# lucidrains/magvit2-pytorch

Hardware: NVIDIA H100
Metric: video-frames/sec tokenize+decode, 17x128x128 bf16 (higher is better)
Workload: dtype bf16

## Files before the change

### magvit2_pytorch_b200/csrc/tc_slab.cu

```cuda
#include "common.cuh"
#include "tc_common.cuh"
#include <cuda.h>
#include <algorithm>
#include <type_traits>
#include <mutex>
#include <map>
#include <vector>
#include <string.h>

namespace mv2 {

struct alignas(64) SlabParams {
  CUtensorMap amap;
  CUtensorMap hmap;
  CUtensorMap wmap;
  CUtensorMap wmap2;
  int kt, kh, kw, pt, ph, pw;
  int st;
  int hist_T;
  int Ci, kchunks, row_bytes;
  int B, T, H, W, Co;
  int mw, pitch, slab_h, slab_bytes, slab_stride;
  int bn, n_tiles_n, tiles_w, tiles_h, total_tiles;
  int slab_stages, w_stages;
  int tpw;
  TcEpi epi;
  CUtensorMap w1map;
  const float* bias1;
  const float* se_wk;
  float se_bk;
  float* se_ws;
  CUtensorMap amap_odd;
  int dn_e_off;
  int dn_aoff[6];
  int dn_lower;
  int h_stride;
  CUtensorMap ymap;
  CUtensorMap rmap;
};

__host__ __device__ constexpr bool slab_tma_epi(int mode) {
  return mode == EPI_PLAIN || mode == EPI_PLAIN_RES || mode == EPI_GEGLU || mode == EPI_DOWN_SPACE;
}
__host__ __device__ constexpr int slab_out_box_ch(int mode, int bn) {
  return (mode == EPI_GEGLU ? bn / 2 : bn) < 64 ? (mode == EPI_GEGLU ? bn / 2 : bn) : 64;
}

__host__ __device__ __forceinline__ void slab_frame_of(const SlabParams& p, int slot, int& b, int& t) {
  const int ptc = p.pt > 0 ? (p.pt + p.st - 1) / p.st : 0;
  const int n_cheap = ptc < p.T ? ptc : p.T, n_full = p.T - n_cheap;
  const int full_slots = p.B * n_full;
  if (slot < full_slots) { b = slot / n_full; t = n_cheap + slot - b * n_full; }
  else { const int r = slot - full_slots; const int level = r / p.B; b = r - level * p.B; t = n_cheap - 1 - level; }
}
__host__ __device__ __forceinline__ int slab_tile_of_cta(const SlabParams& p, int k, int cta, int grid) {
  const int tile = k * grid + ((k & 1) ? grid - 1 - cta : cta);
  return tile < p.total_tiles ? tile : -1;
}
__device__ __forceinline__ int slab_tile_of(const SlabParams& p, int k) { return slab_tile_of_cta(p, k, blockIdx.x, gridDim.x); }

struct TileCoord { int b, t, h0, w0, n0; };
__host__ __device__ __forceinline__ TileCoord decode_tile(const SlabParams& p, int tile) {
  TileCoord c;
  const int nt = tile % p.n_tiles_n; tile /= p.n_tiles_n;
  const int tw = tile % p.tiles_w; tile /= p.tiles_w;
  const int th = tile % p.tiles_h; tile /= p.tiles_h;
  slab_frame_of(p, tile, c.b, c.t);
  c.h0 = th * 16;
  c.w0 = tw * 8 * p.mw;
  c.n0 = nt * p.bn;
  return c;
}

struct SlabSmem { uint32_t sbias, stage0, lpart, accstg, hbuf, end, rbar, otile, rtile; };
__host__ __device__ __forceinline__ SlabSmem slab_smem_layout(const SlabParams& p, uint32_t bar0, bool fused) {
  SlabSmem m;
  m.sbias = (bar0 + 8 * (2 * p.slab_stages + 2 * p.w_stages) + 15) & ~15u;
  m.stage0 = m.sbias + (uint32_t)(p.n_tiles_n * p.bn) * 4 * (fused ? 3 : 1);
  m.lpart = m.stage0 + (fused ? 0 : 8 * 2048);
  m.accstg = m.lpart + (fused ? 2048 : 0);
  m.hbuf = m.accstg + 2u * p.mw * 64 * (p.bn + 4) * 4;
  if (fused) m.hbuf = (m.hbuf + 1023u) & ~1023u;
  m.end = m.hbuf + (fused ? (uint32_t)p.h_stride : 0);
  m.rbar = m.stage0;
  m.otile = (m.rbar + 32 + 1023u) & ~1023u;
  m.rtile = m.otile + 2u * p.mw * 64 * p.bn * 2;
  return m;
}

template <int MODE, int BN, int ACT, int MWMAX>
__device__ __forceinline__ void slab_epi_fragment(const SlabParams& p, const float (&acc)[MWMAX][BN / 2], const TileCoord& c,
                                                  const float* sbias, uint32_t ot, uint32_t rt, int wq, int lane, bool relu) {
  constexpr int OC = MODE == EPI_GEGLU ? BN / 2 : BN, CB = slab_out_box_ch(MODE, BN), NB = OC / CB;
  constexpr uint32_t RB = CB * 2, BOX = 64 * RB, SWZ = (RB / 16 - 1) << 4;
  const uint32_t m0 = 16 * wq + (lane >> 2), q4 = (lane & 3) * 4;
  auto at = [&](int j, int col, uint32_t m) {
    const uint32_t off = m * RB + (uint32_t)(col % CB) * 2 + q4;
    return (uint32_t)(j * NB + col / CB) * BOX + (off ^ ((off >> 3) & SWZ));
  };
  auto st32 = [](uint32_t a, uint32_t v) { asm volatile("st.shared.b32 [%0], %1;" ::"r"(a), "r"(v) : "memory"); };
  const float* os = (MODE == EPI_PLAIN || MODE == EPI_PLAIN_RES) && p.epi.oscale ? p.epi.oscale + (int64_t)c.b * p.Co : nullptr;
  const float rs = MODE == EPI_PLAIN_RES && p.epi.mode == 2 ? 0.70710678118654752440f : 1.f;
#pragma unroll
  for (int j = 0; j < MWMAX; ++j) {
    if (j >= p.mw) break;
    if (MODE == EPI_GEGLU) {
#pragma unroll
      for (int g = 0; g < BN / 16; ++g) {
        const int n = c.n0 + 16 * g + 2 * (lane & 3);
        const float2 bx = *reinterpret_cast<const float2*>(sbias + n), bg = *reinterpret_cast<const float2*>(sbias + n + 8);
#pragma unroll
        for (int hr = 0; hr < 2; ++hr) {
          const float* xv = &acc[j][8 * g + 2 * hr];
          const float* gv = &acc[j][8 * g + 4 + 2 * hr];
          const float v0 = gelu_fast(gv[0] + bg.x) * (xv[0] + bx.x);
          const float v1 = gelu_fast(gv[1] + bg.y) * (xv[1] + bx.y);
          st32(ot + at(j, 8 * g, m0 + 8 * hr), pack_bf16x2(v0, v1));
        }
      }
    } else {
#pragma unroll
      for (int g = 0; g < BN / 8; ++g) {
        const int col = 8 * g, n = c.n0 + col + 2 * (lane & 3);
        const float2 b = *reinterpret_cast<const float2*>(sbias + n);
        float o0 = 1.f, o1 = 1.f;
        if (os) { o0 = n < p.Co ? os[n] : 0.f; o1 = n + 1 < p.Co ? os[n + 1] : 0.f; }
#pragma unroll
        for (int hr = 0; hr < 2; ++hr) {
          float v0 = acc[j][4 * g + 2 * hr], v1 = acc[j][4 * g + 2 * hr + 1];
          if (os) { v0 *= o0; v1 *= o1; }
          v0 = act_ct<ACT>(v0 + b.x, relu);
          v1 = act_ct<ACT>(v1 + b.y, relu);
          const uint32_t a = at(j, col, m0 + 8 * hr);
          if (MODE == EPI_PLAIN_RES) {
            uint32_t r;
            asm volatile("ld.shared.b32 %0, [%1];" : "=r"(r) : "r"(rt + a) : "memory");
            v0 = (v0 + __uint_as_float(r << 16)) * rs;
            v1 = (v1 + __uint_as_float(r & 0xffff0000u)) * rs;
          }
          st32(ot + a, pack_bf16x2(v0, v1));
        }
      }
    }
  }
}

constexpr int SLAB_PRODUCER_REGS = 40, SLAB_CONSUMER_REGS = 232;
template <int MODE, int BN>
__global__ void __launch_bounds__(384, 1) tc_slab_kernel(const __grid_constant__ SlabParams p) {
  constexpr int MWMAX = BN >= 32 ? 128 / BN : 4;
  constexpr int KC1 = BN >= 64 ? BN / 64 : 1;
  extern __shared__ uint8_t smem_raw[];
  const uint32_t smem_base = (smem_u32(smem_raw) + 1023u) & ~1023u;
  const int warp = threadIdx.x >> 5, lane = threadIdx.x & 31;
  const uint32_t row_bytes = p.row_bytes;
  const uint32_t bk = row_bytes >> 1;
  const uint32_t w_tile = p.bn * row_bytes;
  const uint32_t w_bytes = w_tile * p.tpw;
  const uint32_t slab0 = smem_base;
  const uint32_t wst0 = smem_base + p.slab_stages * p.slab_stride;
  const uint32_t bar0 = wst0 + p.w_stages * w_bytes;
  const uint32_t slab_full = bar0, slab_empty = slab_full + 8 * p.slab_stages;
  const uint32_t w_full = slab_empty + 8 * p.slab_stages, w_empty = w_full + 8 * p.w_stages;
  const SlabSmem L = slab_smem_layout(p, bar0, MODE == EPI_FUSED_RU);
  auto gen = [&](uint32_t u) { return smem_raw + (u - smem_u32(smem_raw)); };
  float* sbias = reinterpret_cast<float*>(gen(L.sbias));
  const uint32_t nbias = (uint32_t)(p.n_tiles_n * p.bn);
  const uint32_t stage0 = L.stage0;

  if (threadIdx.x == 0) {
    for (int s = 0; s < p.slab_stages; ++s) { mbar_init(slab_full + 8 * s, 1); mbar_init(slab_empty + 8 * s, 8); }
    for (int s = 0; s < p.w_stages; ++s) { mbar_init(w_full + 8 * s, 1); mbar_init(w_empty + 8 * s, 8); }
    if (MODE == EPI_PLAIN_RES)
      for (int g = 0; g < 2; ++g) { mbar_init(L.rbar + 8 * g, 1); mbar_init(L.rbar + 16 + 8 * g, 4); }
    fence_barrier_init();
  }
  if (warp == 0 && lane == 0) {
    tma_prefetch_desc(&p.amap);
    if (MODE == EPI_DOWN_SPACE) tma_prefetch_desc(&p.amap_odd);
    else if (p.hist_T > 0) tma_prefetch_desc(&p.hmap);
  }
  if (warp == 2 && lane == 0) {
    tma_prefetch_desc(&p.wmap); tma_prefetch_desc(&p.wmap2);
    if (MODE == EPI_FUSED_RU) tma_prefetch_desc(&p.w1map);
  }
  if (slab_tma_epi(MODE) && warp == 1 && lane == 0) {
    tma_prefetch_desc(&p.ymap);
    if (MODE == EPI_PLAIN_RES) tma_prefetch_desc(&p.rmap);
  }
  if (warp >= 4) {
    const int nb = p.n_tiles_n * p.bn;
    for (int i = threadIdx.x - 128; i < nb; i += 256) sbias[i] = (p.epi.bias && i < p.Co) ? p.epi.bias[i] : 0.f;
    if (MODE == EPI_FUSED_RU)
      for (int i = threadIdx.x - 128; i < nb; i += 256) {
        sbias[nb + i] = (p.bias1 && i < p.Co) ? p.bias1[i] : 0.f;
        sbias[2 * nb + i] = i < p.Co ? p.se_wk[i] : 0.f;
      }
  }
  __syncthreads();
  pdl_wait();
  pdl_launch_dependents();

  const int taps2d = p.kh * p.kw;

  if (warp < 4) {
    setmaxnreg_dec<SLAB_PRODUCER_REGS>();
    if (warp == 0) {
      if (MODE == EPI_DOWN_SPACE) {
        if (lane == 0) {
          uint32_t s = 0, ph = 0;
          for (int tk = 0, tile; (tile = slab_tile_of(p, tk)) >= 0; ++tk) {
            const TileCoord c = decode_tile(p, tile);
            for (int kc = 0; kc < p.kchunks; ++kc) {
              mbar_wait(slab_empty + 8 * s, ph ^ 1);
              mbar_expect_tx(slab_full + 8 * s, p.slab_bytes);
              tma_load_5d(slab0 + s * p.slab_stride, &p.amap_odd, slab_full + 8 * s, kc * bk, c.w0 - 1, c.h0 - 1, c.t, c.b);
              tma_load_5d(slab0 + s * p.slab_stride + p.dn_e_off, &p.amap, slab_full + 8 * s, kc * bk, c.w0 - 1, c.h0, c.t, c.b);
              if (++s == (uint32_t)p.slab_stages) { s = 0; ph ^= 1; }
            }
          }
        }
      } else
      if (lane == 0) {
        uint32_t s = 0, ph = 0;
        for (int tk = 0, tile; (tile = slab_tile_of(p, tk)) >= 0; ++tk) {
          const TileCoord c = decode_tile(p, tile);
          const int dt0 = max(0, p.pt - c.t * p.st - p.hist_T);
          for (int dt = dt0; dt < p.kt; ++dt)
            for (int kc = 0; kc < p.kchunks; ++kc) {
              mbar_wait(slab_empty + 8 * s, ph ^ 1);
              mbar_expect_tx(slab_full + 8 * s, p.slab_bytes);
              const int ti = c.t * p.st + dt - p.pt;
              tma_load_5d(slab0 + s * p.slab_stride, ti >= 0 ? &p.amap : &p.hmap, slab_full + 8 * s, kc * bk, c.w0 - p.pw,
                          c.h0 - p.ph, ti >= 0 ? ti : ti + p.hist_T, c.b);
              if (++s == (uint32_t)p.slab_stages) { s = 0; ph ^= 1; }
            }
        }
      }
    } else if (warp == 1) {
// ... 155 lines not shown
                retire_previous(w_last ? w_idx : NONE, w_last && slab_last ? s_idx : NONE);
                accum = 1;
                b_cur += w_tile16;
                if (++dw == p.kw) { dw = 0; a_lo += a_next_dh; } else { a_lo += a_row; }
              }
              next_w_stage();
            }
            if (++s_idx == (uint32_t)p.slab_stages) { s_idx = 0; s_par ^= 1; }
          }
      }
      wgmma_wait<0>();
      release_pending();
    };
    auto mainloop_k = [&](const TileCoord& c, auto mw_c) {
      if (MODE != EPI_FUSED_RU && MODE != EPI_DOWN_SPACE && !k4) mainloop(c, mw_c, std::false_type());
      else mainloop(c, mw_c, std::true_type());
    };
    for (int tk = 0, tile; (tile = slab_tile_of(p, tk)) >= 0; ++tk) {
      const TileCoord c = decode_tile(p, tile);
      if (MWMAX >= 4 && p.mw == 4) mainloop_k(c, std::integral_constant<int, (MWMAX >= 4 ? 4 : 1)>());
      else if (MWMAX >= 2 && p.mw == 2) mainloop_k(c, std::integral_constant<int, (MWMAX >= 2 ? 2 : 1)>());
      else mainloop_k(c, std::integral_constant<int, 1>());
      if (slab_tma_epi(MODE)) {
        constexpr int CB = slab_out_box_ch(MODE, BN), NB = (MODE == EPI_GEGLU ? BN / 2 : BN) / CB;
        constexpr uint32_t BOX = 64 * CB * 2;
        const uint32_t ot = L.otile + (uint32_t)(wg * p.mw * NB) * BOX, rt = L.rtile + (uint32_t)(wg * p.mw) * 64 * BN * 2;
        if (tid == 0) bulk_wait_read_all();
        named_bar_sync(wg_bar, 128);
        if (MODE == EPI_PLAIN_RES) mbar_wait(L.rbar + 8 * wg, r_par);
        const int act = p.epi.act;
        if (MODE == EPI_GEGLU || act == MV2_ACT_NONE)
          slab_epi_fragment<MODE, BN, MV2_ACT_NONE>(p, acc, c, sbias, ot, rt, wq, lane, false);
        else if (act == MV2_ACT_ELU) slab_epi_fragment<MODE, BN, MV2_ACT_ELU>(p, acc, c, sbias, ot, rt, wq, lane, false);
        else if (act == MV2_ACT_SILU) slab_epi_fragment<MODE, BN, MV2_ACT_SILU>(p, acc, c, sbias, ot, rt, wq, lane, false);
        else slab_epi_fragment<MODE, BN, MV2_ACT_LEAKY_RELU>(p, acc, c, sbias, ot, rt, wq, lane, act == MV2_ACT_RELU);
        if (MODE == EPI_PLAIN_RES) {
          __syncwarp();
          if (lane == 0) mbar_arrive(L.rbar + 16 + 8 * wg);
          r_par ^= 1;
        }
        fence_proxy_async();
        named_bar_sync(wg_bar, 128);
        if (tid == 0) {
          const int oc0 = MODE == EPI_GEGLU ? c.n0 / 2 : c.n0, oco = MODE == EPI_GEGLU ? p.Co / 2 : p.Co;
          const int h = c.h0 + 8 * wg;
          for (int j = 0; j < p.mw; ++j)
            for (int b = 0; b < NB; ++b)
              if (h < p.H && c.w0 + 8 * j < p.W && oc0 + b * CB < oco)
                tma_store_5d(&p.ymap, ot + (uint32_t)(j * NB + b) * BOX, oc0 + b * CB, c.w0 + 8 * j, h, c.t, c.b);
          bulk_commit();
        }
        continue;
      }
      named_bar_sync(wg_bar, 128);
#pragma unroll
      for (int j = 0; j < MWMAX; ++j) {
        if (j >= p.mw) break;
        stage_acc<BN>(acc[j], stg + j * 64 * (BN + 4), tid);
      }
      named_bar_sync(wg_bar, 128);
      const int h = c.h0 + lh;
      if (MODE == EPI_FUSED_RU) {
        const float* sb1 = sbias + nbias;
        const float* swk = sbias + 2 * nbias;
        float* lpart = reinterpret_cast<float*>(gen(L.lpart));
        const int64_t kstride = (int64_t)p.W * p.Co;
        const uint32_t wsw = (lane >> 1) & 3;
        const int rl = lane >> 2, piece = lane & 3;
        const int h20 = c.h0 + sub * 4;
        const int recs_per_frame = p.tiles_h * p.tiles_w * 4;
        float* rec = p.se_ws + ((int64_t)(c.b * p.T + c.t) * recs_per_frame + ((c.h0 >> 4) * p.tiles_w + c.w0 / (8 * p.mw)) * 4 + sub) * (p.Co + 2);
        float run_m = -INFINITY, run_s = 0.f, run_acc[2][8];
#pragma unroll
        for (int q = 0; q < 2; ++q)
#pragma unroll
          for (int i = 0; i < 8; ++i) run_acc[q][i] = 0.f;
        const uint64_t h_hi = gmma_desc_hi(1024, 128);
        const uint32_t h_lo = desc_lo(L.hbuf) + (uint32_t)wg * ((64 * 128) >> 4);
        uint32_t w1_slot[KC1], w1_par[KC1], w1_lo[KC1];
#pragma unroll
        for (int kc2 = 0; kc2 < KC1; ++kc2) {
          w1_slot[kc2] = w_idx; w1_par[kc2] = w_par; w1_lo[kc2] = b_lo;
          if (++w_idx == (uint32_t)p.w_stages) { w_idx = 0; w_par ^= 1; b_lo = b_lo0; } else { b_lo += w_stage16; }
        }
        for (int j = 0; j < p.mw; ++j) {
          const float* srow = stg + (j * 64 + row - 64 * wg) * (BN + 4);
          const uint32_t stg2 = smem_u32(stg + (j * 64 + (sub & 1) * 32) * (BN + 4)) + (uint32_t)half * 2048;
          const uint32_t wr = stg2 + lane * 64, rd = stg2 + rl * 64;
          const uint32_t hb = L.hbuf + (uint32_t)row * 128;
          for (int c0 = half * 32; c0 < p.bn; c0 += 64) {
            uint32_t r[32], pk[16];
            load_row32(srow + c0, 32, r);
            epi_pack32_t<MV2_ACT_ELU>(r, sbias + c0, pk);
            const uint32_t hrow = hb + (uint32_t)(c0 >> 6) * 16384;
            const uint32_t p0 = (uint32_t)(c0 & 63) >> 3;
#pragma unroll
            for (int g = 0; g < 4; ++g)
              asm volatile("st.shared.v4.b32 [%0], {%1, %2, %3, %4};" ::"r"(hrow + (((p0 + g) ^ ((uint32_t)row & 7u)) << 4)),
                           "r"(pk[4 * g]), "r"(pk[4 * g + 1]), "r"(pk[4 * g + 2]), "r"(pk[4 * g + 3]) : "memory");
          }
          fence_proxy_async();
          named_bar_sync(wg_bar, 128);
#pragma unroll
          for (int kc2 = 0; kc2 < KC1; ++kc2) mbar_wait(w_full + 8 * w1_slot[kc2], w1_par[kc2]);
          wgmma_fence();
#pragma unroll
          for (int kc2 = 0; kc2 < KC1; ++kc2) {
            const uint64_t ad = h_hi | (uint64_t)(h_lo + kc2 * (16384 >> 4)), bd = h_hi | (uint64_t)w1_lo[kc2];
            wgmma_bf16<BN>(acc[0], ad, bd, kc2 > 0 ? 1u : 0u);
            wgmma_bf16<BN>(acc[0], ad + 2, bd + 2, 1u);
            wgmma_bf16<BN>(acc[0], ad + 4, bd + 4, 1u);
            wgmma_bf16<BN>(acc[0], ad + 6, bd + 6, 1u);
          }
          wgmma_commit();
          wgmma_wait<0>();
          if (j == p.mw - 1) {
            __syncwarp();
            if (lane == 0)
#pragma unroll
              for (int kc2 = 0; kc2 < KC1; ++kc2) mbar_arrive(w_empty + 8 * w1_slot[kc2]);
          }
          stage_acc<BN>(acc[0], stg + j * 64 * (BN + 4), tid);
          named_bar_sync(wg_bar, 128);
          const int w = c.w0 + 8 * j + lw;
          const bool row_ok = h < p.H && w < p.W;
          uint32_t pk2[2][16];
          float lp = 0.f;
#pragma unroll
          for (int q = 0; q < 2; ++q) {
            const int c0 = half * 32 + 64 * q;
            if (c0 < p.bn) {
              uint32_t r[32];
              load_row32(srow + c0, 32, r);
              epi_pack32_t<MV2_ACT_ELU>(r, sb1 + c0, pk2[q]);
#pragma unroll
              for (int i = 0; i < 16; i += 2) {
                const float4 wv = *reinterpret_cast<const float4*>(swk + c0 + 2 * i);
                lp = fmaf(__uint_as_float(pk2[q][i] << 16), wv.x, lp);
                lp = fmaf(__uint_as_float(pk2[q][i] & 0xffff0000u), wv.y, lp);
                lp = fmaf(__uint_as_float(pk2[q][i + 1] << 16), wv.z, lp);
                lp = fmaf(__uint_as_float(pk2[q][i + 1] & 0xffff0000u), wv.w, lp);
              }
            }
          }
          float* lpb = lpart + (ecount & 1u) * 256;
          ++ecount;
          lpb[ew * 32 + lane] = lp;
          asm volatile("bar.sync %0, 64;" ::"r"(1 + sub) : "memory");
          float lg = lpb[sub * 32 + lane] + lpb[(sub + 4) * 32 + lane] + p.se_bk;
          lg = row_ok ? lg : -INFINITY;
          const float mx = warp_max(lg);
          const float ev = lg > -INFINITY ? ex2_approx((lg - mx) * 1.4426950408889634f) : 0.f;
          const float es = warp_sum(ev);
          float e4[4];
#pragma unroll
          for (int k = 0; k < 4; ++k) e4[k] = __shfl_sync(0xffffffffu, ev, 8 * k + rl);
          const float new_m = fmaxf(run_m, mx);
          const float ca = run_m > -INFINITY ? ex2_approx((run_m - new_m) * 1.4426950408889634f) : 0.f;
          const float cb = mx > -INFINITY ? ex2_approx((mx - new_m) * 1.4426950408889634f) : 0.f;
          run_s = fmaf(run_s, ca, es * cb);
          run_m = new_m;
          const int w2 = c.w0 + 8 * j + rl;
          const int64_t row0 = ((((int64_t)c.b * p.T + c.t) * p.H + h20) * p.W + w2) * p.Co + piece * 8;
          const int kmax = w2 < p.W ? p.H - h20 : 0;
#pragma unroll
          for (int q = 0; q < 2; ++q) {
            const int c0 = half * 32 + 64 * q;
            if (c0 < p.bn) {
#pragma unroll
              for (int g = 0; g < 4; ++g)
                asm volatile("st.shared.v4.b32 [%0], {%1, %2, %3, %4};" ::"r"(wr + ((g ^ wsw) << 4)), "r"(pk2[q][4 * g]),
                             "r"(pk2[q][4 * g + 1]), "r"(pk2[q][4 * g + 2]), "r"(pk2[q][4 * g + 3]) : "memory");
              __syncwarp();
              __nv_bfloat16* yp = p.epi.y + row0 + c0;
              float t[8];
#pragma unroll
              for (int i = 0; i < 8; ++i) t[i] = 0.f;
#pragma unroll
              for (int k = 0; k < 4; ++k) {
                uint4 v;
                asm volatile("ld.shared.v4.b32 {%0, %1, %2, %3}, [%4];" : "=r"(v.x), "=r"(v.y), "=r"(v.z), "=r"(v.w)
                             : "r"(rd + k * 512 + ((piece ^ (((8 * k + rl) >> 1) & 3)) << 4)));
                if (k < kmax) *reinterpret_cast<uint4*>(yp + k * kstride) = v;
                const uint32_t vv[4] = {v.x, v.y, v.z, v.w};
#pragma unroll
                for (int i = 0; i < 4; ++i) {
                  t[2 * i] = fmaf(e4[k], __uint_as_float(vv[i] << 16), t[2 * i]);
                  t[2 * i + 1] = fmaf(e4[k], __uint_as_float(vv[i] & 0xffff0000u), t[2 * i + 1]);
                }
              }
              __syncwarp();
#pragma unroll
              for (int i = 0; i < 8; ++i) {
                t[i] += __shfl_xor_sync(0xffffffffu, t[i], 4);
                t[i] += __shfl_xor_sync(0xffffffffu, t[i], 8);
                t[i] += __shfl_xor_sync(0xffffffffu, t[i], 16);
              }
#pragma unroll
              for (int i = 0; i < 8; ++i) run_acc[q][i] = fmaf(run_acc[q][i], ca, t[i] * cb);
            }
          }
        }
        if (half == 0 && lane == 0) { rec[0] = run_m; rec[1] = run_s; }
        if (rl == 0) {
#pragma unroll
          for (int q = 0; q < 2; ++q) {
            const int c0 = half * 32 + 64 * q;
            if (c0 < p.bn) {
              float2* dst = reinterpret_cast<float2*>(rec + 2 + c0 + piece * 8);
              dst[0] = make_float2(run_acc[q][0], run_acc[q][1]); dst[1] = make_float2(run_acc[q][2], run_acc[q][3]);
              dst[2] = make_float2(run_acc[q][4], run_acc[q][5]); dst[3] = make_float2(run_acc[q][6], run_acc[q][7]);
            }
          }
        }
      } else
      for (int j = 0; j < p.mw; ++j) {
        const int w = c.w0 + 8 * j + lw;
        const bool row_ok = h < p.H && w < p.W;
        const float* srow = stg + (j * 64 + row - 64 * wg) * (BN + 4);
        const int64_t row_base = ((((int64_t)c.b * p.T + c.t) * p.H + h) * p.W + w) * p.Co;
        if (MODE == EPI_SHUFFLE_ST) {
          const uint32_t stg = stage0 + (uint32_t)ew * 2048;
          const uint32_t wr = stg + lane * 64, wsw = (lane >> 1) & 3;
          const int rl = lane >> 2, piece = lane & 3;
          const int w2 = c.w0 + 8 * j + rl;
          const uint32_t rd = stg + rl * 64;
          const int h20 = c.h0 + sub * 4;
          const int kmax = w2 < p.W ? p.H - h20 : 0;
          for (int c0 = ((j + half) & 1) * 32; c0 < p.bn; c0 += 64) {
            uint32_t r[32], pk[16];
            load_row32(srow + c0, 32, r);
            epi_pack32(p.epi.act, r, sbias + c.n0 + c0, pk);
#pragma unroll
            for (int g = 0; g < 4; ++g)
              asm volatile("st.shared.v4.b32 [%0], {%1, %2, %3, %4};" ::"r"(wr + ((g ^ wsw) << 4)), "r"(pk[4 * g]),
                           "r"(pk[4 * g + 1]), "r"(pk[4 * g + 2]), "r"(pk[4 * g + 3]) : "memory");
            __syncwarp();
            const bool col_ok = c.n0 + c0 + piece * 8 < p.Co && c0 + piece * 8 < p.bn;
            const int klim = col_ok ? kmax : 0;
            __nv_bfloat16* yp;
            int64_t ks;
            const int n = c.n0 + c0;
            if (p.epi.shuffle == MV2_SHUFFLE_SPACE) {
              const int cy = p.Co >> 2, qd = n / cy, cb = n - qd * cy;
              yp = p.epi.y + ((((int64_t)c.b * p.T + c.t) * (2 * p.H) + (2 * h20 + (qd >> 1))) * (2 * p.W) + (2 * w2 + (qd & 1))) * cy + cb + piece * 8;
              ks = (int64_t)4 * p.W * cy;
            } else {
              const int cy = p.Co >> 1, qd = n / cy, cb = n - qd * cy;
              yp = p.epi.y + ((((int64_t)c.b * (2 * p.T) + (2 * c.t + qd)) * p.H + h20) * p.W + w2) * cy + cb + piece * 8;
              ks = (int64_t)p.W * cy;
            }
#pragma unroll
            for (int k = 0; k < 4; ++k) {
              uint4 v;
              asm volatile("ld.shared.v4.b32 {%0, %1, %2, %3}, [%4];" : "=r"(v.x), "=r"(v.y), "=r"(v.z), "=r"(v.w)
                           : "r"(rd + k * 512 + ((piece ^ (((8 * k + rl) >> 1) & 3)) << 4)));
              if (k < klim) *reinterpret_cast<uint4*>(yp + k * ks) = v;
            }
            __syncwarp();
          }
        } else {
          for (int c0 = ((j + half) & 1) * 32; c0 < p.bn; c0 += 64) {
            uint32_t r[32];
            load_row32(srow + c0, BN < 32 ? BN : 32, r);
            if (row_ok) epi_chunk32<MODE>(p.epi, r, min(32, p.bn - c0), c.n0 + c0, sbias + c.n0 + c0, c.b, c.t, h, w, row_base);
          }
        }
      }
    }
    if (slab_tma_epi(MODE) && tid == 0) bulk_wait_all();
  }
}

}

using namespace mv2;

static bool slab_narrow(const mv2_tc_conv_args* a) { return a->out_layout == 1 && a->Co <= 16 && a->kw > 3; }

extern "C" int mv2_tc_slab_supported(const mv2_tc_conv_args* a) {
  if (!a) return 0;
  if (a->sh != 1 || a->sw != 1) return 0;
  if (a->st != 1) {
    if (a->st != 2 || a->out_layout != 0 || a->epi_mode != 0 || a->shuffle != MV2_SHUFFLE_NONE) return 0;
    if (a->To != (a->Ti + a->pt - a->kt) / a->st + 1 || a->To < 1) return 0;
  }
  if (a->Ci % 32 != 0 || a->Co > 4096) return 0;
  if (a->oscale && (a->epi_mode != 0 || a->shuffle != MV2_SHUFFLE_NONE)) return 0;
  if (a->epi_mode == 1 && (a->Co % 64 != 0 || a->shuffle != MV2_SHUFFLE_NONE || a->res)) return 0;
  if (a->epi_mode == 2 && (!a->res || a->shuffle != MV2_SHUFFLE_NONE)) return 0;
  if (a->epi_mode < 0 || a->epi_mode > 2) return 0;
  if (a->Co % 32 != 0 && a->Co > 32) return 0;
  if (a->Ci % 64 != 0 && a->kw != 1) return 0;
  if (a->res && a->Co % 8 != 0) return 0;
  if (a->shuffle != MV2_SHUFFLE_NONE && ((a->shuffle == MV2_SHUFFLE_SPACE ? a->Co / 4 : a->Co / 2) % 8 != 0 || a->Co % 32 != 0)) return 0;
  if (a->kh > 7 || a->kw > (slab_narrow(a) ? 7 : 3) || a->kt > 8) return 0;
  if (a->Ho != a->Hi || a->Wo != a->Wi) return 0;
  if (a->out_layout == 1) {
    if (a->Co % 8 == 0 || a->res || a->shuffle != MV2_SHUFFLE_NONE || a->epi_mode != 0) return 0;
    if (a->To > a->Ti || a->To < 1) return 0;
    if (a->pt != a->kt - 1 - (a->Ti - a->To) && a->pt != -(a->Ti - a->To)) return 0;
  } else if (a->out_layout != 0 || (a->st == 1 && a->To != a->Ti)) return 0;
  return 1;
}

static int slab_ring_budget(const SlabParams& p, bool fused) {
  SlabParams q = p;
  q.slab_stages = 3; q.w_stages = 12;
  return 227 * 1024 - 2048 - (int)slab_smem_layout(q, 0, fused).end;
}
static size_t slab_smem_bytes(const SlabParams& p, bool fused) {
  const uint32_t rings = (uint32_t)(p.slab_stages * p.slab_stride + p.w_stages * p.bn * p.row_bytes * p.tpw);
  return 1024 + slab_smem_layout(p, rings, fused).end;
}
static int slab_default_mw(int bn, int Wo) { return bn <= 32 && Wo > 16 ? 4 : (bn <= 64 && Wo > 8 ? 2 : 1); }
static void slab_set_geometry(SlabParams& p, int mw) {
  p.mw = mw;
  p.pitch = 8 * mw + p.kw - 1;
  p.slab_bytes = p.pitch * p.slab_h * p.row_bytes;
  p.slab_stride = (p.slab_bytes + 1023) / 1024 * 1024;
  p.tiles_w = ceil_div(p.W, 8 * mw);
  p.total_tiles = (int)((int64_t)p.B * p.T * p.tiles_h * p.tiles_w * p.n_tiles_n);
}
// ... 127 lines not shown
  if (tile >= 0) {
    const TileCoord c = decode_tile(p, tile);
    out6[1] = c.b; out6[2] = c.t; out6[3] = c.h0; out6[4] = c.w0; out6[5] = c.n0;
  }
  return MV2_OK;
}

extern "C" int mv2_tc_slab_forward(const mv2_tc_conv_args* a, const mv2_conv_hist* hist, void* stream) {
  MV2_CHECK_ARG(a && a->x && a->w && a->y);
  MV2_CHECK_ARG(!hist || (hist->T_h >= 0 && (hist->T_h == 0 || (hist->h && hist->clip_stride > 0))));
  if (!mv2_tc_slab_supported(a)) { set_error("mv2_tc_slab_forward: unsupported shape"); return MV2_E_UNSUPPORTED; }
  SlabParams p;
  if (const int rc = slab_fill_plan(a, p)) return rc;
  if (const int rc = slab_encode_maps(p, a, hist)) return rc;
  int mode = EPI_PLAIN;
  if (a->epi_mode == 1) mode = EPI_GEGLU;
  else if (a->shuffle != MV2_SHUFFLE_NONE && (a->Co / (a->shuffle == MV2_SHUFFLE_SPACE ? 4 : 2)) % 32 == 0) mode = EPI_SHUFFLE_ST;
  else if (a->shuffle != MV2_SHUFFLE_NONE) mode = EPI_SHUFFLE;
  else if (a->Co % 8 != 0) mode = EPI_RAGGED;
  else if (a->res) mode = EPI_PLAIN_RES;
  if (slab_tma_epi(mode))
    if (const int rc = slab_encode_out_maps(p, mode)) return rc;
  return slab_launch(mode, p, stream);
}


static void ru_as_conv_args(const mv2_tc_ru_args* a, mv2_tc_conv_args* c) {
  memset(c, 0, sizeof(*c));
  c->x = a->x; c->w = a->w3; c->bias = a->b3; c->res = nullptr; c->y = a->y;
  c->B = a->B; c->Ti = c->To = a->T; c->Hi = c->Ho = a->H; c->Wi = c->Wo = a->W; c->Ci = c->Co = a->C;
  c->kt = a->kt; c->kh = a->kh; c->kw = a->kw; c->st = c->sh = c->sw = 1;
  c->pt = a->kt - 1; c->ph = a->kh / 2; c->pw = a->kw / 2;
  c->act = MV2_ACT_ELU; c->shuffle = MV2_SHUFFLE_NONE; c->epi_mode = 0;
}

extern "C" int mv2_tc_ru_supported(const mv2_tc_ru_args* a) {
  if (!a) return 0;
  if (a->C != 64 && a->C != 128) return 0;
  if (a->W <= 8) return 0;
  if (a->kt < 1 || a->kt > 8 || a->kh < 1 || a->kh > 7 || a->kw < 1 || a->kw > 3) return 0;
  if ((a->kh & 1) == 0 || (a->kw & 1) == 0) return 0;
  mv2_tc_conv_args c;
  ru_as_conv_args(a, &c);
  return mv2_tc_slab_supported(&c);
}

static int ru_fill_plan(const mv2_tc_ru_args* a, SlabParams& p) {
  mv2_tc_conv_args c;
  ru_as_conv_args(a, &c);
  if (const int rc = slab_fill_plan(&c, p)) return rc;
  MV2_CHECK_ARG(p.bn == a->C && p.n_tiles_n == 1 && p.row_bytes == 128);
  p.tpw = 1;
  p.h_stride = p.kchunks * 16384;
  const int budget = slab_ring_budget(p, true);
  p.slab_stages = 2;
  p.w_stages = std::min(12, (budget - 2 * p.slab_stride) / (p.bn * p.row_bytes));
  MV2_CHECK_ARG(p.w_stages >= 2);
  p.bias1 = a->b1; p.se_wk = a->se_wk; p.se_bk = a->se_bk; p.se_ws = a->se_ws;
  return MV2_OK;
}

extern "C" int mv2_tc_ru_records(const mv2_tc_ru_args* a) {
  if (!mv2_tc_ru_supported(a)) { set_error("mv2_tc_ru_records: unsupported shape"); return MV2_E_UNSUPPORTED; }
  SlabParams p;
  if (const int rc = ru_fill_plan(a, p)) return rc;
  return p.tiles_h * p.tiles_w * 4;
}

extern "C" size_t mv2_tc_ru_workspace_bytes(const mv2_tc_ru_args* a) {
  const int recs = mv2_tc_ru_records(a);
  if (recs <= 0) return 0;
  const size_t F = (size_t)a->B * a->T;
  return (F * recs * (a->C + 2) + F * (a->C + 16)) * sizeof(float);
}

extern "C" int mv2_tc_ru_forward(const mv2_tc_ru_args* a, const mv2_conv_hist* hist, void* stream) {
  MV2_CHECK_ARG(a && a->x && a->w3 && a->w1 && a->y && a->se_wk && a->se_ws);
  MV2_CHECK_ARG(!hist || (hist->T_h >= 0 && (hist->T_h == 0 || (hist->h && hist->clip_stride > 0))));
  if (!mv2_tc_ru_supported(a)) { set_error("mv2_tc_ru_forward: unsupported shape"); return MV2_E_UNSUPPORTED; }
  SlabParams p;
  if (const int rc = ru_fill_plan(a, p)) return rc;
  mv2_tc_conv_args c;
  ru_as_conv_args(a, &c);
  if (const int rc = slab_encode_maps(p, &c, hist)) return rc;
  const cuuint64_t dims1[2] = {(cuuint64_t)a->C, (cuuint64_t)a->C};
  const cuuint64_t strides1[1] = {(cuuint64_t)a->C * 2};
  const cuuint32_t box1[2] = {64, (cuuint32_t)p.bn};
  if (const int rc = encode_bf16_map(&p.w1map, 2, a->w1, dims1, strides1, box1, CU_TENSOR_MAP_SWIZZLE_128B, "w1")) return rc;
  return slab_launch(EPI_FUSED_RU, p, stream);
}


extern "C" int mv2_tc_down_space_supported(const mv2_tc_conv_args* a) {
  if (!a) return 0;
  if (a->kt != 1 || a->kh != 3 || a->kw != 3 || a->st != 1 || a->sh != 2 || a->sw != 2) return 0;
  if (a->pt != 0 || a->ph != 1 || a->pw != 1) return 0;
  if ((a->Hi & 1) || (a->Wi & 1) || a->Ho != a->Hi / 2 || a->Wo != a->Wi / 2 || a->To != a->Ti) return 0;
  if (a->Ci % 64 != 0 || a->Co % 32 != 0 || a->Co > 4096) return 0;
  if (a->res || a->shuffle != MV2_SHUFFLE_NONE || a->epi_mode != 0 || a->out_layout != 0 || a->oscale) return 0;
  return 1;
}

extern "C" int mv2_tc_down_space_forward(const mv2_tc_conv_args* a, void* stream) {
  MV2_CHECK_ARG(a && a->x && a->w && a->y);
  if (!mv2_tc_down_space_supported(a)) { set_error("mv2_tc_down_space_forward: unsupported shape"); return MV2_E_UNSUPPORTED; }
  SlabParams p;
  memset(&p, 0, sizeof(p));
  const int C2 = 2 * a->Ci, bk = 64;
  p.kt = 1; p.kh = 3; p.kw = 2; p.pt = 0; p.ph = 1; p.pw = 1; p.st = 1;
  p.row_bytes = 128; p.Ci = C2; p.kchunks = C2 / bk; p.dn_lower = a->Ci / bk;
  p.B = a->B; p.T = a->To; p.H = a->Ho; p.W = a->Wo; p.Co = a->Co;
  p.epi = tc_epi_of(a);
  int bn = 32;
  for (int c = 128; c >= 32; c >>= 1) if (a->Co % c == 0) { bn = c; break; }
  const int w_bytes = bn * 128;
  p.bn = bn; p.n_tiles_n = a->Co / bn; p.tpw = 1;
  p.tiles_h = ceil_div(a->Ho, 16);
  p.slab_h = 17;
  int budget;
  for (int mw = slab_default_mw(bn, a->Wo);; mw >>= 1) {
    slab_set_geometry(p, mw);
    p.dn_e_off = p.slab_stride;
    const int e_bytes = 16 * p.pitch * 128;
    p.slab_bytes += e_bytes;
    p.slab_stride += (e_bytes + 1023) / 1024 * 1024;
    budget = slab_ring_budget(p, false);
    if (mw == 1 || 2 * p.slab_stride + 3 * w_bytes <= budget) break;
  }
  for (int dh = 0; dh < 3; ++dh)
    for (int q = 0; q < 2; ++q)
      p.dn_aoff[dh * 2 + q] = ((dh == 1 ? p.dn_e_off : 0) + ((dh == 2 ? p.pitch : 0) + q) * 128) >> 4;
  p.slab_stages = p.slab_stride * 3 + w_bytes * 4 <= budget ? 3 : 2;
  p.w_stages = std::min(12, (budget - p.slab_stages * p.slab_stride) / w_bytes);
  MV2_CHECK_ARG(p.w_stages >= 2);

  const int64_t rowb = (int64_t)a->Wi * a->Ci * 2;
  const cuuint64_t dims[5] = {(cuuint64_t)C2, (cuuint64_t)(a->Wi / 2), (cuuint64_t)(a->Hi / 2), (cuuint64_t)a->Ti, (cuuint64_t)a->B};
  const cuuint64_t strides[4] = {(cuuint64_t)(C2 * 2), (cuuint64_t)(2 * rowb), (cuuint64_t)(a->Hi * rowb), (cuuint64_t)(a->Ti * a->Hi * rowb)};
  const cuuint32_t box_e[5] = {(cuuint32_t)bk, (cuuint32_t)p.pitch, 16, 1, 1}, box_o[5] = {(cuuint32_t)bk, (cuuint32_t)p.pitch, 17, 1, 1};
  if (const int rc = encode_bf16_map(&p.amap, 5, a->x, dims, strides, box_e, CU_TENSOR_MAP_SWIZZLE_128B, "even rows")) return rc;
  if (const int rc = encode_bf16_map(&p.amap_odd, 5, (const char*)a->x + rowb, dims, strides, box_o, CU_TENSOR_MAP_SWIZZLE_128B, "odd rows")) return rc;
// ... 10 lines not shown
```

Measured before the change: 5203.

## Route fused residual-unit epilogue through register-direct swizzled tiles and TMA stores

The fused residual-unit path no longer stages fp32 accumulators through a padded shared buffer. It writes ELU-activated bf16 fragments straight into swizzled smem tiles that feed the second GEMM and the output, stores the output with TMA bulk stores, and reads the SE-pooling inputs back from the output tile. This removes an fp32 staging round trip, a named barrier and the per-thread global stores. Freeing the staging space lets the plan use three slab stages when the budget allows. The cost is a different smem layout and extra bulk-store waits.

```diff
diff --git a/magvit2_pytorch_b200/csrc/tc_slab.cu b/magvit2_pytorch_b200/csrc/tc_slab.cu
--- a/magvit2_pytorch_b200/csrc/tc_slab.cu
+++ b/magvit2_pytorch_b200/csrc/tc_slab.cu
@@ -74,74 +74,84 @@
 
 struct SlabSmem { uint32_t sbias, stage0, lpart, accstg, hbuf, end, rbar, otile, rtile; };
 __host__ __device__ __forceinline__ SlabSmem slab_smem_layout(const SlabParams& p, uint32_t bar0, bool fused) {
-  SlabSmem m;
+  SlabSmem m = {};
   m.sbias = (bar0 + 8 * (2 * p.slab_stages + 2 * p.w_stages) + 15) & ~15u;
   m.stage0 = m.sbias + (uint32_t)(p.n_tiles_n * p.bn) * 4 * (fused ? 3 : 1);
-  m.lpart = m.stage0 + (fused ? 0 : 8 * 2048);
-  m.accstg = m.lpart + (fused ? 2048 : 0);
-  m.hbuf = m.accstg + 2u * p.mw * 64 * (p.bn + 4) * 4;
-  if (fused) m.hbuf = (m.hbuf + 1023u) & ~1023u;
-  m.end = m.hbuf + (fused ? (uint32_t)p.h_stride : 0);
+  if (fused) {
+    m.lpart = m.stage0;
+    m.hbuf = (m.lpart + 2048 + 1023u) & ~1023u;
+    m.otile = m.hbuf + (uint32_t)p.h_stride;
+    m.end = m.otile + 2u * p.mw * 64 * p.bn * 2;
+    return m;
+  }
+  m.accstg = m.stage0 + 8 * 2048;
+  m.end = m.accstg + 2u * p.mw * 64 * (p.bn + 4) * 4;
   m.rbar = m.stage0;
   m.otile = (m.rbar + 32 + 1023u) & ~1023u;
   m.rtile = m.otile + 2u * p.mw * 64 * p.bn * 2;
   return m;
 }
 
-template <int MODE, int BN, int ACT, int MWMAX>
-__device__ __forceinline__ void slab_epi_fragment(const SlabParams& p, const float (&acc)[MWMAX][BN / 2], const TileCoord& c,
-                                                  const float* sbias, uint32_t ot, uint32_t rt, int wq, int lane, bool relu) {
-  constexpr int OC = MODE == EPI_GEGLU ? BN / 2 : BN, CB = slab_out_box_ch(MODE, BN), NB = OC / CB;
+template <int MODE, int BN, int ACT>
+__device__ __forceinline__ void slab_epi_mtile(const SlabParams& p, const float (&acc)[BN / 2], const TileCoord& c,
+                                               const float* sbias, uint32_t ot, uint32_t rt, int wq, int lane, bool relu) {
+  constexpr int CB = slab_out_box_ch(MODE, BN);
   constexpr uint32_t RB = CB * 2, BOX = 64 * RB, SWZ = (RB / 16 - 1) << 4;
   const uint32_t m0 = 16 * wq + (lane >> 2), q4 = (lane & 3) * 4;
-  auto at = [&](int j, int col, uint32_t m) {
+  auto at = [&](int col, uint32_t m) {
     const uint32_t off = m * RB + (uint32_t)(col % CB) * 2 + q4;
-    return (uint32_t)(j * NB + col / CB) * BOX + (off ^ ((off >> 3) & SWZ));
+    return (uint32_t)(col / CB) * BOX + (off ^ ((off >> 3) & SWZ));
   };
   auto st32 = [](uint32_t a, uint32_t v) { asm volatile("st.shared.b32 [%0], %1;" ::"r"(a), "r"(v) : "memory"); };
   const float* os = (MODE == EPI_PLAIN || MODE == EPI_PLAIN_RES) && p.epi.oscale ? p.epi.oscale + (int64_t)c.b * p.Co : nullptr;
   const float rs = MODE == EPI_PLAIN_RES && p.epi.mode == 2 ? 0.70710678118654752440f : 1.f;
+  if (MODE == EPI_GEGLU) {
+#pragma unroll
+    for (int g = 0; g < BN / 16; ++g) {
+      const int n = c.n0 + 16 * g + 2 * (lane & 3);
+      const float2 bx = *reinterpret_cast<const float2*>(sbias + n), bg = *reinterpret_cast<const float2*>(sbias + n + 8);
+#pragma unroll
+      for (int hr = 0; hr < 2; ++hr) {
+        const float* xv = &acc[8 * g + 2 * hr];
+        const float* gv = &acc[8 * g + 4 + 2 * hr];
+        const float v0 = gelu_fast(gv[0] + bg.x) * (xv[0] + bx.x);
+        const float v1 = gelu_fast(gv[1] + bg.y) * (xv[1] + bx.y);
+        st32(ot + at(8 * g, m0 + 8 * hr), pack_bf16x2(v0, v1));
+      }
+    }
+  } else {
+#pragma unroll
+    for (int g = 0; g < BN / 8; ++g) {
+      const int col = 8 * g, n = c.n0 + col + 2 * (lane & 3);
+      const float2 b = *reinterpret_cast<const float2*>(sbias + n);
+      float o0 = 1.f, o1 = 1.f;
+      if (os) { o0 = n < p.Co ? os[n] : 0.f; o1 = n + 1 < p.Co ? os[n + 1] : 0.f; }
+#pragma unroll
+      for (int hr = 0; hr < 2; ++hr) {
+        float v0 = acc[4 * g + 2 * hr], v1 = acc[4 * g + 2 * hr + 1];
+        if (os) { v0 *= o0; v1 *= o1; }
+        v0 = act_ct<ACT>(v0 + b.x, relu);
+        v1 = act_ct<ACT>(v1 + b.y, relu);
+        const uint32_t a = at(col, m0 + 8 * hr);
+        if (MODE == EPI_PLAIN_RES) {
+          uint32_t r;
+          asm volatile("ld.shared.b32 %0, [%1];" : "=r"(r) : "r"(rt + a) : "memory");
+          v0 = (v0 + __uint_as_float(r << 16)) * rs;
+          v1 = (v1 + __uint_as_float(r & 0xffff0000u)) * rs;
+        }
+        st32(ot + a, pack_bf16x2(v0, v1));
+      }
+    }
+  }
+}
+template <int MODE, int BN, int ACT, int MWMAX>
+__device__ __forceinline__ void slab_epi_fragment(const SlabParams& p, const float (&acc)[MWMAX][BN / 2], const TileCoord& c,
+                                                  const float* sbias, uint32_t ot, uint32_t rt, int wq, int lane, bool relu) {
+  constexpr uint32_t MTILE = (MODE == EPI_GEGLU ? BN / 2 : BN) * 64 * 2;
 #pragma unroll
   for (int j = 0; j < MWMAX; ++j) {
     if (j >= p.mw) break;
-    if (MODE == EPI_GEGLU) {
-#pragma unroll
-      for (int g = 0; g < BN / 16; ++g) {
-        const int n = c.n0 + 16 * g + 2 * (lane & 3);
-        const float2 bx = *reinterpret_cast<const float2*>(sbias + n), bg = *reinterpret_cast<const float2*>(sbias + n + 8);
-#pragma unroll
-        for (int hr = 0; hr < 2; ++hr) {
-          const float* xv = &acc[j][8 * g + 2 * hr];
-          const float* gv = &acc[j][8 * g + 4 + 2 * hr];
-          const float v0 = gelu_fast(gv[0] + bg.x) * (xv[0] + bx.x);
-          const float v1 = gelu_fast(gv[1] + bg.y) * (xv[1] + bx.y);
-          st32(ot + at(j, 8 * g, m0 + 8 * hr), pack_bf16x2(v0, v1));
-        }
-      }
-    } else {
-#pragma unroll
-      for (int g = 0; g < BN / 8; ++g) {
-        const int col = 8 * g, n = c.n0 + col + 2 * (lane & 3);
-        const float2 b = *reinterpret_cast<const float2*>(sbias + n);
-        float o0 = 1.f, o1 = 1.f;
-        if (os) { o0 = n < p.Co ? os[n] : 0.f; o1 = n + 1 < p.Co ? os[n + 1] : 0.f; }
-#pragma unroll
-        for (int hr = 0; hr < 2; ++hr) {
-          float v0 = acc[j][4 * g + 2 * hr], v1 = acc[j][4 * g + 2 * hr + 1];
-          if (os) { v0 *= o0; v1 *= o1; }
-          v0 = act_ct<ACT>(v0 + b.x, relu);
-          v1 = act_ct<ACT>(v1 + b.y, relu);
-          const uint32_t a = at(j, col, m0 + 8 * hr);
-          if (MODE == EPI_PLAIN_RES) {
-            uint32_t r;
-            asm volatile("ld.shared.b32 %0, [%1];" : "=r"(r) : "r"(rt + a) : "memory");
-            v0 = (v0 + __uint_as_float(r << 16)) * rs;
-            v1 = (v1 + __uint_as_float(r & 0xffff0000u)) * rs;
-          }
-          st32(ot + a, pack_bf16x2(v0, v1));
-        }
-      }
-    }
+    slab_epi_mtile<MODE, BN, ACT>(p, acc[j], c, sbias, ot + j * MTILE, rt + j * MTILE, wq, lane, relu);
   }
 }
 
@@ -150,6 +160,7 @@
 __global__ void __launch_bounds__(384, 1) tc_slab_kernel(const __grid_constant__ SlabParams p) {
   constexpr int MWMAX = BN >= 32 ? 128 / BN : 4;
   constexpr int KC1 = BN >= 64 ? BN / 64 : 1;
+  constexpr bool TMA_STORE = slab_tma_epi(MODE) || MODE == EPI_FUSED_RU;
   extern __shared__ uint8_t smem_raw[];
   const uint32_t smem_base = (smem_u32(smem_raw) + 1023u) & ~1023u;
   const int warp = threadIdx.x >> 5, lane = threadIdx.x & 31;
@@ -184,7 +195,7 @@
     tma_prefetch_desc(&p.wmap); tma_prefetch_desc(&p.wmap2);
     if (MODE == EPI_FUSED_RU) tma_prefetch_desc(&p.w1map);
   }
-  if (slab_tma_epi(MODE) && warp == 1 && lane == 0) {
+  if (TMA_STORE && warp == 1 && lane == 0) {
     tma_prefetch_desc(&p.ymap);
     if (MODE == EPI_PLAIN_RES) tma_prefetch_desc(&p.rmap);
   }
@@ -446,22 +457,16 @@
         }
         continue;
       }
-      named_bar_sync(wg_bar, 128);
-#pragma unroll
-      for (int j = 0; j < MWMAX; ++j) {
-        if (j >= p.mw) break;
-        stage_acc<BN>(acc[j], stg + j * 64 * (BN + 4), tid);
-      }
-      named_bar_sync(wg_bar, 128);
-      const int h = c.h0 + lh;
       if (MODE == EPI_FUSED_RU) {
+        constexpr int CB = slab_out_box_ch(MODE, BN), NB = BN / CB;
+        constexpr uint32_t BOX = 64 * CB * 2;
         const float* sb1 = sbias + nbias;
         const float* swk = sbias + 2 * nbias;
         float* lpart = reinterpret_cast<float*>(gen(L.lpart));
-        const int64_t kstride = (int64_t)p.W * p.Co;
-        const uint32_t wsw = (lane >> 1) & 3;
+        const uint32_t hb = L.hbuf + (uint32_t)wg * KC1 * BOX, ot = L.otile + (uint32_t)(wg * p.mw * NB) * BOX;
+        const int h = c.h0 + lh;
         const int rl = lane >> 2, piece = lane & 3;
-        const int h20 = c.h0 + sub * 4;
+        const uint32_t mrow = (uint32_t)(row & 63), mq = mrow & ~31u;
         const int recs_per_frame = p.tiles_h * p.tiles_w * 4;
         float* rec = p.se_ws + ((int64_t)(c.b * p.T + c.t) * recs_per_frame + ((c.h0 >> 4) * p.tiles_w + c.w0 / (8 * p.mw)) * 4 + sub) * (p.Co + 2);
         float run_m = -INFINITY, run_s = 0.f, run_acc[2][8];
@@ -470,29 +475,18 @@
 #pragma unroll
           for (int i = 0; i < 8; ++i) run_acc[q][i] = 0.f;
         const uint64_t h_hi = gmma_desc_hi(1024, 128);
-        const uint32_t h_lo = desc_lo(L.hbuf) + (uint32_t)wg * ((64 * 128) >> 4);
+        const uint32_t h_lo = desc_lo(hb);
         uint32_t w1_slot[KC1], w1_par[KC1], w1_lo[KC1];
 #pragma unroll
         for (int kc2 = 0; kc2 < KC1; ++kc2) {
           w1_slot[kc2] = w_idx; w1_par[kc2] = w_par; w1_lo[kc2] = b_lo;
           if (++w_idx == (uint32_t)p.w_stages) { w_idx = 0; w_par ^= 1; b_lo = b_lo0; } else { b_lo += w_stage16; }
         }
-        for (int j = 0; j < p.mw; ++j) {
-          const float* srow = stg + (j * 64 + row - 64 * wg) * (BN + 4);
-          const uint32_t stg2 = smem_u32(stg + (j * 64 + (sub & 1) * 32) * (BN + 4)) + (uint32_t)half * 2048;
-          const uint32_t wr = stg2 + lane * 64, rd = stg2 + rl * 64;
-          const uint32_t hb = L.hbuf + (uint32_t)row * 128;
-          for (int c0 = half * 32; c0 < p.bn; c0 += 64) {
-            uint32_t r[32], pk[16];
-            load_row32(srow + c0, 32, r);
-            epi_pack32_t<MV2_ACT_ELU>(r, sbias + c0, pk);
-            const uint32_t hrow = hb + (uint32_t)(c0 >> 6) * 16384;
-            const uint32_t p0 = (uint32_t)(c0 & 63) >> 3;
-#pragma unroll
-            for (int g = 0; g < 4; ++g)
-              asm volatile("st.shared.v4.b32 [%0], {%1, %2, %3, %4};" ::"r"(hrow + (((p0 + g) ^ ((uint32_t)row & 7u)) << 4)),
-                           "r"(pk[4 * g]), "r"(pk[4 * g + 1]), "r"(pk[4 * g + 2]), "r"(pk[4 * g + 3]) : "memory");
-          }
+        if (tid == 0) bulk_wait_read_all();
+#pragma unroll
+        for (int j = 0; j < MWMAX; ++j) {
+          if (j >= p.mw) break;
+          slab_epi_mtile<MODE, BN, MV2_ACT_ELU>(p, acc[j], c, sbias, hb, 0, wq, lane, false);
           fence_proxy_async();
           named_bar_sync(wg_bar, 128);
 #pragma unroll
@@ -500,7 +494,7 @@
           wgmma_fence();
 #pragma unroll
           for (int kc2 = 0; kc2 < KC1; ++kc2) {
-            const uint64_t ad = h_hi | (uint64_t)(h_lo + kc2 * (16384 >> 4)), bd = h_hi | (uint64_t)w1_lo[kc2];
+            const uint64_t ad = h_hi | (uint64_t)(h_lo + kc2 * (BOX >> 4)), bd = h_hi | (uint64_t)w1_lo[kc2];
             wgmma_bf16<BN>(acc[0], ad, bd, kc2 > 0 ? 1u : 0u);
             wgmma_bf16<BN>(acc[0], ad + 2, bd + 2, 1u);
             wgmma_bf16<BN>(acc[0], ad + 4, bd + 4, 1u);
@@ -514,29 +508,41 @@
 #pragma unroll
               for (int kc2 = 0; kc2 < KC1; ++kc2) mbar_arrive(w_empty + 8 * w1_slot[kc2]);
           }
-          stage_acc<BN>(acc[0], stg + j * 64 * (BN + 4), tid);
+          const uint32_t otj = ot + (uint32_t)(j * NB) * BOX;
+          slab_epi_mtile<MODE, BN, MV2_ACT_ELU>(p, acc[0], c, sb1, otj, 0, wq, lane, false);
+          fence_proxy_async();
           named_bar_sync(wg_bar, 128);
+          if (tid == 0) {
+            if (c.h0 + 8 * wg < p.H && c.w0 + 8 * j < p.W)
+#pragma unroll
+              for (int b = 0; b < NB; ++b) tma_store_5d(&p.ymap, otj + (uint32_t)b * BOX, b * CB, c.w0 + 8 * j, c.h0 + 8 * wg, c.t, c.b);
+            bulk_commit();
+          }
+          auto ld_y = [&](int q, uint32_t m, uint32_t u) {
+            uint4 v;
+            asm volatile("ld.shared.v4.b32 {%0, %1, %2, %3}, [%4];" : "=r"(v.x), "=r"(v.y), "=r"(v.z), "=r"(v.w)
+                         : "r"(otj + (uint32_t)q * BOX + m * 128 + ((u ^ (m & 7)) << 4)) : "memory");
+            return v;
+          };
           const int w = c.w0 + 8 * j + lw;
           const bool row_ok = h < p.H && w < p.W;
-          uint32_t pk2[2][16];
           float lp = 0.f;
 #pragma unroll
-          for (int q = 0; q < 2; ++q) {
-            const int c0 = half * 32 + 64 * q;
-            if (c0 < p.bn) {
-              uint32_t r[32];
-              load_row32(srow + c0, 32, r);
-              epi_pack32_t<MV2_ACT_ELU>(r, sb1 + c0, pk2[q]);
-#pragma unroll
-              for (int i = 0; i < 16; i += 2) {
-                const float4 wv = *reinterpret_cast<const float4*>(swk + c0 + 2 * i);
-                lp = fmaf(__uint_as_float(pk2[q][i] << 16), wv.x, lp);
-                lp = fmaf(__uint_as_float(pk2[q][i] & 0xffff0000u), wv.y, lp);
-                lp = fmaf(__uint_as_float(pk2[q][i + 1] << 16), wv.z, lp);
-                lp = fmaf(__uint_as_float(pk2[q][i + 1] & 0xffff0000u), wv.w, lp);
-              }
+          for (int q = 0; q < NB; ++q)
+#pragma unroll
+            for (int g = 0; g < 4; ++g) {
+              const uint4 v = ld_y(q, mrow, 4 * half + g);
+              const float4 wa = *reinterpret_cast<const float4*>(swk + half * 32 + 64 * q + 8 * g);
+              const float4 wb = *reinterpret_cast<const float4*>(swk + half * 32 + 64 * q + 8 * g + 4);
+              lp = fmaf(__uint_as_float(v.x << 16), wa.x, lp);
+              lp = fmaf(__uint_as_float(v.x & 0xffff0000u), wa.y, lp);
+              lp = fmaf(__uint_as_float(v.y << 16), wa.z, lp);
+              lp = fmaf(__uint_as_float(v.y & 0xffff0000u), wa.w, lp);
+              lp = fmaf(__uint_as_float(v.z << 16), wb.x, lp);
+              lp = fmaf(__uint_as_float(v.z & 0xffff0000u), wb.y, lp);
+              lp = fmaf(__uint_as_float(v.w << 16), wb.z, lp);
+              lp = fmaf(__uint_as_float(v.w & 0xffff0000u), wb.w, lp);
             }
-          }
           float* lpb = lpart + (ecount & 1u) * 256;
           ++ecount;
           lpb[ew * 32 + lane] = lp;
@@ -554,60 +560,50 @@
           const float cb = mx > -INFINITY ? ex2_approx((mx - new_m) * 1.4426950408889634f) : 0.f;
           run_s = fmaf(run_s, ca, es * cb);
           run_m = new_m;
-          const int w2 = c.w0 + 8 * j + rl;
-          const int64_t row0 = ((((int64_t)c.b * p.T + c.t) * p.H + h20) * p.W + w2) * p.Co + piece * 8;
-          const int kmax = w2 < p.W ? p.H - h20 : 0;
-#pragma unroll
-          for (int q = 0; q < 2; ++q) {
-            const int c0 = half * 32 + 64 * q;
-            if (c0 < p.bn) {
-#pragma unroll
-              for (int g = 0; g < 4; ++g)
-                asm volatile("st.shared.v4.b32 [%0], {%1, %2, %3, %4};" ::"r"(wr + ((g ^ wsw) << 4)), "r"(pk2[q][4 * g]),
-                             "r"(pk2[q][4 * g + 1]), "r"(pk2[q][4 * g + 2]), "r"(pk2[q][4 * g + 3]) : "memory");
-              __syncwarp();
-              __nv_bfloat16* yp = p.epi.y + row0 + c0;
-              float t[8];
-#pragma unroll
-              for (int i = 0; i < 8; ++i) t[i] = 0.f;
-#pragma unroll
-              for (int k = 0; k < 4; ++k) {
-                uint4 v;
-                asm volatile("ld.shared.v4.b32 {%0, %1, %2, %3}, [%4];" : "=r"(v.x), "=r"(v.y), "=r"(v.z), "=r"(v.w)
-                             : "r"(rd + k * 512 + ((piece ^ (((8 * k + rl) >> 1) & 3)) << 4)));
-                if (k < kmax) *reinterpret_cast<uint4*>(yp + k * kstride) = v;
-                const uint32_t vv[4] = {v.x, v.y, v.z, v.w};
-#pragma unroll
-                for (int i = 0; i < 4; ++i) {
-                  t[2 * i] = fmaf(e4[k], __uint_as_float(vv[i] << 16), t[2 * i]);
-                  t[2 * i + 1] = fmaf(e4[k], __uint_as_float(vv[i] & 0xffff0000u), t[2 * i + 1]);
-                }
+#pragma unroll
+          for (int q = 0; q < NB; ++q) {
+            float t[8];
+#pragma unroll
+            for (int i = 0; i < 8; ++i) t[i] = 0.f;
+#pragma unroll
+            for (int k = 0; k < 4; ++k) {
+              const uint4 v = ld_y(q, mq + 8 * k + rl, 4 * half + piece);
+              const uint32_t vv[4] = {v.x, v.y, v.z, v.w};
+#pragma unroll
+              for (int i = 0; i < 4; ++i) {
+                t[2 * i] = fmaf(e4[k], __uint_as_float(vv[i] << 16), t[2 * i]);
+                t[2 * i + 1] = fmaf(e4[k], __uint_as_float(vv[i] & 0xffff0000u), t[2 * i + 1]);
               }
-              __syncwarp();
-#pragma unroll
-              for (int i = 0; i < 8; ++i) {
-                t[i] += __shfl_xor_sync(0xffffffffu, t[i], 4);
-                t[i] += __shfl_xor_sync(0xffffffffu, t[i], 8);
-                t[i] += __shfl_xor_sync(0xffffffffu, t[i], 16);
-              }
-#pragma unroll
-              for (int i = 0; i < 8; ++i) run_acc[q][i] = fmaf(run_acc[q][i], ca, t[i] * cb);
             }
+#pragma unroll
+            for (int i = 0; i < 8; ++i) {
+              t[i] += __shfl_xor_sync(0xffffffffu, t[i], 4);
+              t[i] += __shfl_xor_sync(0xffffffffu, t[i], 8);
+              t[i] += __shfl_xor_sync(0xffffffffu, t[i], 16);
+            }
+#pragma unroll
+            for (int i = 0; i < 8; ++i) run_acc[q][i] = fmaf(run_acc[q][i], ca, t[i] * cb);
           }
         }
         if (half == 0 && lane == 0) { rec[0] = run_m; rec[1] = run_s; }
         if (rl == 0) {
 #pragma unroll
-          for (int q = 0; q < 2; ++q) {
-            const int c0 = half * 32 + 64 * q;
-            if (c0 < p.bn) {
-              float2* dst = reinterpret_cast<float2*>(rec + 2 + c0 + piece * 8);
-              dst[0] = make_float2(run_acc[q][0], run_acc[q][1]); dst[1] = make_float2(run_acc[q][2], run_acc[q][3]);
-              dst[2] = make_float2(run_acc[q][4], run_acc[q][5]); dst[3] = make_float2(run_acc[q][6], run_acc[q][7]);
-            }
-          }
-        }
-      } else
+          for (int q = 0; q < NB; ++q) {
+            float2* dst = reinterpret_cast<float2*>(rec + 2 + half * 32 + 64 * q + piece * 8);
+            dst[0] = make_float2(run_acc[q][0], run_acc[q][1]); dst[1] = make_float2(run_acc[q][2], run_acc[q][3]);
+            dst[2] = make_float2(run_acc[q][4], run_acc[q][5]); dst[3] = make_float2(run_acc[q][6], run_acc[q][7]);
+          }
+        }
+        continue;
+      }
+      named_bar_sync(wg_bar, 128);
+#pragma unroll
+      for (int j = 0; j < MWMAX; ++j) {
+        if (j >= p.mw) break;
+        stage_acc<BN>(acc[j], stg + j * 64 * (BN + 4), tid);
+      }
+      named_bar_sync(wg_bar, 128);
+      const int h = c.h0 + lh;
       for (int j = 0; j < p.mw; ++j) {
         const int w = c.w0 + 8 * j + lw;
         const bool row_ok = h < p.H && w < p.W;
@@ -662,7 +658,7 @@
         }
       }
     }
-    if (slab_tma_epi(MODE) && tid == 0) bulk_wait_all();
+    if (TMA_STORE && tid == 0) bulk_wait_all();
   }
 }
 
@@ -896,9 +892,9 @@
   MV2_CHECK_ARG(p.bn == a->C && p.n_tiles_n == 1 && p.row_bytes == 128);
   p.tpw = 1;
   p.h_stride = p.kchunks * 16384;
-  const int budget = slab_ring_budget(p, true);
-  p.slab_stages = 2;
-  p.w_stages = std::min(12, (budget - 2 * p.slab_stride) / (p.bn * p.row_bytes));
+  const int budget = slab_ring_budget(p, true), w_bytes = p.bn * p.row_bytes;
+  p.slab_stages = 3 * p.slab_stride + 2 * w_bytes <= budget ? 3 : 2;
+  p.w_stages = std::min(12, (budget - p.slab_stages * p.slab_stride) / w_bytes);
   MV2_CHECK_ARG(p.w_stages >= 2);
   p.bias1 = a->b1; p.se_wk = a->se_wk; p.se_bk = a->se_bk; p.se_ws = a->se_ws;
   return MV2_OK;
@@ -931,6 +927,7 @@
   const cuuint64_t strides1[1] = {(cuuint64_t)a->C * 2};
   const cuuint32_t box1[2] = {64, (cuuint32_t)p.bn};
   if (const int rc = encode_bf16_map(&p.w1map, 2, a->w1, dims1, strides1, box1, CU_TENSOR_MAP_SWIZZLE_128B, "w1")) return rc;
+  if (const int rc = slab_encode_out_maps(p, EPI_FUSED_RU)) return rc;
   return slab_launch(EPI_FUSED_RU, p, stream);
 }
 
```

New measurement: 5513, median of 6. 6.0% higher.
